# MGI-tech-bioinformatics/SuperPlus

Measured on AMD Instinct MI355X. Metric: k-mers/s (DF createDict stage: trim + canonical k-mer count + solid filter + spectrum + adjacency), higher is better.
Workload: dtype u64

## Files before the change

superplus_amd/csrc/dfk.hip:

```cpp
#include "../../include/dfk.h"
#include "dfk_kernels.h"
#include "dfk_arena.h"

#include <algorithm>
#include <chrono>
#include <cstdarg>
#include <cstdio>
#include <cstdlib>
#include <cstring>
#include <atomic>
#include <fcntl.h>
#include <functional>
#include <new>
#include <string>
#include <sys/mman.h>
#include <sys/stat.h>
#include <unistd.h>
#include <condition_variable>
#include <memory>
#include <mutex>
#include <numeric>
#include <thread>
#include <vector>

// ... 346 lines not shown
        HIP_TRY(hipStreamWaitEvent(ks, J->ev_scan, 0));
        if (step.wait_prev_count) HIP_TRY(hipStreamWaitEvent(ks, J->ev_count, 0));
    }
    HIP_TRY(hipMemsetAsync(cnt, 0, n_subs * 8, ks));
    const dim3 per_class(std::max(1u, 16u * cus / P.n_cls), P.n_cls);
    const uint32_t sh = 6 + P.sb;
    hipLaunchKernelGGL(k_keys_subcount, per_class, dim3(256), P.n_sub * 4, ks,
                       (const uint32_t*)sk.keys, (const unsigned long long*)sk.fill, sk.cap, sh, P.n_sub, cnt);
    HIP_TRY(hipGetLastError());
    hipLaunchKernelGGL(k_keys_offsets, dim3(1), dim3(1024), 0, ks, (const unsigned long long*)cnt, (uint32_t)n_subs, off, cur);
    HIP_TRY(hipGetLastError());
    hipLaunchKernelGGL(k_keys_partition, per_class, dim3(256), P.n_sub * 12, ks,
                       (const uint32_t*)sk.keys, (const unsigned long long*)sk.fill, sk.cap, sh, P.n_sub, cur, (uint32_t*)J->keys2.p);
    HIP_TRY(hipGetLastError());
    if (two) HIP_TRY(hipEventRecord(J->ev_part[sl], ks));
    ++J->n_pieces; J->count_due = true;
    if (!two) return scan_keys_count(c, T, J);
    return 0;
}

template <int K>
int scan_range(dfk_ctx* c, const Inputs& in, BucketTable* T, ScanJob* J, uint64_t r0, uint64_t r1)
{
    if (r1 <= r0) return 0;
    const PartParams& pp = J->pp;
    const ScanPlan& P = J->plan;
    const unsigned grid = scan_grid(P, r1 - r0, (unsigned)c->prop.multiProcessorCount);
    hipEvent_t e0, e1;
    HIP_TRY(hipEventCreate(&e0)); HIP_TRY(hipEventCreate(&e1));
    J->ev.emplace_back(e0, e1);
    HIP_TRY(hipEventRecord(e0, c->stream));
    if (P.keyed) {
        uint64_t p0 = r0;
        for (uint64_t m : scan_piece_sizes(P, r1 - r0, r1 == in.n_reads)) {
            int rc = scan_keys_piece<K>(c, in, T, J, p0, p0 + m); if (rc) return rc;
            p0 += m;
        }
        if (r1 == in.n_reads && J->count_due) { int rc = scan_keys_count(c, T, J); if (rc) return rc; }
    } else if (P.register_scan) {
        hipLaunchKernelGGL(HIP_KERNEL_NAME(k_scan_count<K, 16, false>), dim3(grid), dim3(PART_THREADS), scan_lds(P), c->stream,
                           in.packed, in.packed_bytes, in.base_off, (const uint32_t*)c->good_len.p, r0, r1, pp,
                           (unsigned long long*)T->acc.p, (unsigned long long*)T->class_hist.p, (unsigned long long*)J->d_n.p, P.ovf_cap,
                           (uint32_t*)J->ovf_tmp.p, (uint4*)T->summ.p, (uint32_t*)T->classes.p, ScanKeys{});
    } else {
        if (r0 != 0 || r1 != in.n_reads) return fail(DFK_E_STATE, "the general scan takes every read at once");
        hipLaunchKernelGGL(HIP_KERNEL_NAME(k_partition<K, false>), dim3(grid), dim3(PART_THREADS), scan_lds(P), c->stream,
                           in.packed, in.packed_bytes, in.base_off, (const uint32_t*)c->good_len.p, in.bc,
                           (int64_t)c->cfg.ign_bc_below, in.n_reads, pp, (unsigned long long*)T->acc.p, (unsigned long long*)T->class_hist.p,
                           (unsigned long long*)J->d_n.p, P.ovf_cap, (uint4*)J->ovf_tmp.p, (uint4*)T->summ.p,
                           (const uint32_t*)nullptr, (uint64_t)0, (const uint64_t*)nullptr, (uint32_t*)T->classes.p);
    }
    HIP_TRY(hipGetLastError());
    HIP_TRY(hipEventRecord(e1, c->stream));
    return 0;
}

template <int K>
int scan_end(dfk_ctx* c, const Inputs& in, uint64_t n_inst, BucketTable* T, ScanJob* J)
{
    int rc = 0;
    T->n_ovf = 0;
    if (J->count_due) { rc = scan_keys_count(c, T, J); if (rc) return rc; }
    c->release(J->keys); c->release(J->keys2); c->release(J->fill); c->release(J->sub);
    if (in.n_reads) {
        HIP_TRY(hipMemcpyAsync(&T->n_ovf, J->d_n.p, 8, hipMemcpyDeviceToHost, c->stream));
        HIP_TRY(hipStreamSynchronize(c->stream));
        if (T->n_ovf > J->plan.ovf_cap) {
            c->release(J->ovf_tmp);
            rc = c->alloc(J->ovf_tmp, in.n_reads * 4, "overflow read list (scratch)"); if (rc) return rc;
            HIP_TRY(hipMemsetAsync(J->d_n.p, 0, 16, c->stream));
            hipLaunchKernelGGL(k_select_overflow, dim3((unsigned)std::min<uint64_t>((in.n_reads + 255) / 256, 8192)), dim3(256), 0, c->stream,
                               (const uint4*)T->summ.p, in.n_reads, (uint32_t*)J->ovf_tmp.p, (unsigned long long*)J->d_n.p);
            HIP_TRY(hipGetLastError());
            HIP_TRY(hipMemcpyAsync(&T->n_ovf, J->d_n.p, 8, hipMemcpyDeviceToHost, c->stream));
            HIP_TRY(hipStreamSynchronize(c->stream));
        }
        if (T->n_ovf) {
            rc = c->alloc(T->ovf_list, T->n_ovf * 4, "overflow read list", Place::Low); if (rc) return rc;
            HIP_TRY(hipMemcpyAsync(T->ovf_list.p, J->ovf_tmp.p, T->n_ovf * 4, hipMemcpyDeviceToDevice, c->stream));
            HIP_TRY(hipStreamSynchronize(c->stream));
        }
    }
    c->release(J->ovf_tmp); c->release(J->d_n);
    HIP_TRY(hipStreamSynchronize(c->stream));
    float ms = 0;
    for (auto& e : J->ev) { float m = 0; if (hipEventElapsedTime(&m, e.first, e.second) == hipSuccess) ms += m; }
    c->st.ms_part_count = ms; c->st.reserved[6] = J->ev.size();
    TRACE("%llu of %llu reads have more than %d runs", (unsigned long long)T->n_ovf, (unsigned long long)in.n_reads, SUMMARY_RUNS);
    const uint64_t nb = J->plan.nb, n_bins = J->plan.n_bins;
    if (J->plan.by_class) {
        T->h_class.assign(n_bins, 0);
        HIP_TRY(hipMemcpyAsync(T->h_class.data(), T->class_hist.p, n_bins * 8, hipMemcpyDeviceToHost, c->stream));
        HIP_TRY(hipStreamSynchronize(c->stream));
        T->n_records = T->n_inst = 0;
        for (uint64_t i = 0; i < n_bins / 2; ++i) { T->n_records += T->h_class[i]; T->n_inst += T->h_class[n_bins / 2 + i]; }
    } else { rc = table_totals(c, T->acc, nb, &T->n_records, &T->n_inst); if (rc) return rc; }
    TRACE("partition count pass done (%llu buckets, %llu records%s)", (unsigned long long)nb, (unsigned long long)T->n_records, J->ev.size() > 1 ? ", in ranges under the upload" : "");
    if (T->n_inst != n_inst)
        return fail(DFK_E_HIP, "partition count pass saw %llu instances, trim saw %llu%s",
                    (unsigned long long)T->n_inst, (unsigned long long)n_inst,
                    (n_inst - T->n_inst) % (1ull << 32) == 0 ? " (a fine bucket with 2^32 or more instances: its counter keeps 32 bits)" : "");
    c->st.n_records = T->n_records; c->st.n_buckets = nb;
    return 0;
}

template <int K>
int partition_count(dfk_ctx* c, const Inputs& in, uint64_t n_inst, uint32_t log2_world, int64_t read_id0, BucketTable* T, bool by_class = false)
{
    ScanJob J;
    int rc = scan_begin<K>(c, in, log2_world, read_id0, T, by_class, &J); if (rc) return rc;
    rc = scan_range<K>(c, in, T, &J, 0, in.n_reads); if (rc) return rc;
    return scan_end<K>(c, in, n_inst, T, &J);
}

int pass_tables(dfk_ctx* c, const DevBuf& acc, uint32_t log2_sub, uint32_t world, uint32_t sub_lo, uint32_t sub_n, uint64_t budget, Partition* P)
{
    P->nb = (uint64_t)world * sub_n;
    const uint64_t nb = P->nb;
    DevBuf rec, inst, flags, idx;
    int rc = c->alloc(rec, (nb + 1) * 8, "bucket record counts"); if (rc) return rc;
    rc = c->alloc(inst, (nb + 1) * 8, "bucket instance counts"); if (rc) return rc;
    rc = c->alloc(P->base, (nb + 1) * 8, "bucket bases"); if (rc) return rc;
    rc = c->alloc(P->ipre, (nb + 1) * 8, "bucket instance prefix"); if (rc) return rc;
    const unsigned g1 = (unsigned)((nb + 1 + 255) / 256);
    hipLaunchKernelGGL(k_slice, dim3(g1), dim3(256), 0, c->stream, (const unsigned long long*)acc.p, log2_sub, sub_lo, sub_n, nb,
                       (uint64_t*)rec.p, (uint64_t*)inst.p);
    HIP_TRY(hipGetLastError());
    rc = device_scan(c, (const uint64_t*)rec.p, (uint64_t*)P->base.p, nb + 1); if (rc) return rc;
    rc = device_scan(c, (const uint64_t*)inst.p, (uint64_t*)P->ipre.p, nb + 1); if (rc) return rc;
    rc = c->alloc(flags, (nb + 1) * 8, "item flags"); if (rc) return rc;
    rc = c->alloc(idx, (nb + 1) * 8, "item index"); if (rc) return rc;
    hipLaunchKernelGGL(k_item_flags, dim3(g1), dim3(256), 0, c->stream, (const uint64_t*)P->ipre.p, nb, budget, (uint64_t*)flags.p);
    HIP_TRY(hipGetLastError());
    rc = device_scan(c, (const uint64_t*)flags.p, (uint64_t*)idx.p, nb + 1); if (rc) return rc;
    uint64_t tot[3];
    HIP_TRY(hipMemcpyAsync(&tot[0], (const uint64_t*)P->base.p + nb, 8, hipMemcpyDeviceToHost, c->stream));
    HIP_TRY(hipMemcpyAsync(&tot[1], (const uint64_t*)P->ipre.p + nb, 8, hipMemcpyDeviceToHost, c->stream));
    HIP_TRY(hipMemcpyAsync(&tot[2], (const uint64_t*)idx.p + nb, 8, hipMemcpyDeviceToHost, c->stream));
    HIP_TRY(hipStreamSynchronize(c->stream));
    P->n_records = tot[0]; P->n_inst = tot[1]; P->n_items = tot[2];
    rc = c->alloc(P->items, std::max<uint64_t>(1, P->n_items) * sizeof(ItemRange), "work items"); if (rc) return rc;
    hipLaunchKernelGGL(k_item_pairs, dim3((unsigned)((nb + 255) / 256)), dim3(256), 0, c->stream, (const uint64_t*)flags.p,
                       (const uint64_t*)idx.p, nb, (ItemRange*)P->items.p);
    HIP_TRY(hipGetLastError());
    HIP_TRY(hipStreamSynchronize(c->stream));
    c->release(rec); c->release(inst); c->release(flags); c->release(idx);
    return 0;
}

void release_pass(dfk_ctx* c, Partition* P)
{ c->release(P->records); c->release(P->base); c->release(P->ipre); c->release(P->items); }

template <int K> uint64_t item_budget(const dfk_ctx* c)
{
    constexpr uint64_t S = 1ull << CountCfg<K>::LOG2S;
    if (c->cfg.inst_per_item) return c->cfg.inst_per_item;
    if (c->distinct_per_inst <= 0.0) return 3 * S / 2;
    const double b = 0.367 * (double)S / c->distinct_per_inst;
    return (uint64_t)std::min(std::max(b, 0.5 * (double)S), 3.0 * (double)S);
}

struct ScatterJob { Partition P; DevBuf cur, d_bad; hipStream_t st = nullptr; hipEvent_t e0 = nullptr, e1 = nullptr; uint32_t lo = 0, n = 0; };

template <int K>
int scatter_launch(dfk_ctx* c, const Inputs& in, const BucketTable& T, uint32_t log2_world, int64_t read_id0, ScatterJob* J)
{
    const PartParams pp = part_params<K>(c, T.log2_nb, log2_world, read_id0, J->lo, J->n);
    HIP_TRY(hipEventRecord(J->e0, J->st));
    if (in.n_reads)
        hipLaunchKernelGGL(HIP_KERNEL_NAME(k_scatter_runs<K>), dim3((unsigned)((in.n_reads + 256ull * sweep_reads<K>() - 1) / (256ull * sweep_reads<K>()))),
                           dim3(256), 0, J->st,
// ... 1423 lines not shown
```

superplus_amd/csrc/dfk_kernels.h:

```cpp
#pragma once
#include <type_traits>
#include "dfk_device.h"
#include "dfk_fallback.h"
#include "dfk_scan_plan.h"

namespace dfk {

template <int K>
__global__ void __launch_bounds__(256)
k_trim(const uint8_t* __restrict__ pq, const uint64_t* __restrict__ pq_off, uint64_t pq_nbytes,
       const uint64_t* __restrict__ base_off, uint64_t packed_bytes, const uint32_t* __restrict__ read_len,
       uint64_t n_reads, uint32_t min_qual, uint32_t* __restrict__ good_len,
       unsigned long long* __restrict__ n_inst, unsigned int* __restrict__ bad,
       unsigned long long* __restrict__ sum_good)
{
    unsigned long long mine = 0, good = 0;
    bool any_bad = false;
    for (uint64_t r = (uint64_t)blockIdx.x * blockDim.x + threadIdx.x; r < n_reads; r += (uint64_t)gridDim.x * blockDim.x) {
        uint32_t gl = 0;
        uint64_t p = pq_off[r], end = pq_off[r + 1];
        uint32_t idx = 0, run = 0;
        const uint64_t b0 = base_off[r], b1 = base_off[r + 1];
        bool ok = p <= end && end <= pq_nbytes && b0 <= b1 && b1 <= packed_bytes && b1 - b0 >= ((uint64_t)read_len[r] + 3) / 4;
        if (!ok) end = p;
        while (p < end) {
            uint32_t nQs = pq[p];
            if (!nQs) break;
            if (p + 3 > end) { ok = false; break; }
            uint32_t hdr = pq[p + 1] | ((uint32_t)pq[p + 2] << 8);
            uint32_t nBits = hdr & 7u, minQ = (hdr >> 3) & 63u;
            uint64_t blk = ((uint64_t)nQs * nBits + 24) >> 3;
            if (p + blk > end) { ok = false; break; }
            if (nBits == 0) {
                if (minQ >= min_qual) { run += nQs; if (run >= (uint32_t)K) gl = idx + nQs; }
                else run = 0;
                idx += nQs;
            } else {
                uint64_t bit = 8 * (p + 1) + 9;
                const uint32_t fmask = (1u << nBits) - 1u;
                for (uint32_t left = nQs; left;) {
                    const uint64_t by = bit >> 3;
                    const uint32_t sh = (uint32_t)(bit & 7);
                    uint64_t w = 0;
                    if (by + 8 <= pq_nbytes) __builtin_memcpy(&w, pq + by, 8);
                    else for (uint32_t k = 0; k < 8 && by + k < pq_nbytes; ++k) w |= (uint64_t)pq[by + k] << (8 * k);
                    w >>= sh;
                    const uint32_t n = min(left, (64u - sh) / nBits);
                    for (uint32_t i = 0; i < n; ++i, w >>= nBits) {
                        const uint32_t q = minQ + ((uint32_t)w & fmask);
                        if (q < min_qual) run = 0;
                        else if (++run >= (uint32_t)K) gl = idx + 1;
                        ++idx;
                    }
                    bit += (uint64_t)n * nBits; left -= n;
                }
            }
            p += blk;
        }
        uint32_t rl = read_len[r];
        if (!ok || idx != rl) { any_bad = true; gl = 0; }
        if (gl > rl) gl = rl;
        good_len[r] = gl;
        good += gl;
        if (gl >= (uint32_t)K + 1) mine += gl - K + 1;
    }
    __shared__ unsigned long long sh[2][4];
    __shared__ unsigned int sh_bad;
    if (threadIdx.x == 0) sh_bad = 0;
    __syncthreads();
#pragma unroll
    for (int d = 32; d > 0; d >>= 1) { mine += __shfl_down(mine, d, 64); good += __shfl_down(good, d, 64); }
    if ((threadIdx.x & 63) == 0) { sh[0][threadIdx.x >> 6] = mine; sh[1][threadIdx.x >> 6] = good; }
    if (any_bad) atomicOr(&sh_bad, 1u);
    __syncthreads();
    if (threadIdx.x == 0) {
        unsigned long long a0 = sh[0][0] + sh[0][1] + sh[0][2] + sh[0][3], a1 = sh[1][0] + sh[1][1] + sh[1][2] + sh[1][3];
        if (a0) atomicAdd(n_inst, a0);
        if (a1) atomicAdd(sum_good, a1);
        if (sh_bad) atomicOr(bad, 1u);
    }
}

struct PartParams {
    uint32_t M;
    uint32_t W;
    uint32_t log2_nb;
// ... 13 lines not shown
    const uint32_t a = sweep_class_of(sub_lo, log2_local), b = sweep_class_of(sub_lo + sub_n - 1, log2_local);
    const uint32_t upto_b = b >= 31 ? 0xFFFFFFFFu : ((1u << (b + 1)) - 1u);
    return upto_b & ~((1u << a) - 1u);
}

constexpr uint32_t SUMMARY_OVERFLOW = 15;

__device__ __forceinline__ uint32_t pass_local(uint32_t bucket, const PartParams& pp)
{
    const uint32_t ls = pp.log2_nb - pp.log2_world;
    const uint32_t d = (bucket & ((1u << ls) - 1u)) - pp.sub_lo;
    return d < pp.sub_n ? (bucket >> ls) * pp.sub_n + d : 0xFFFFFFFFu;
}

__device__ __forceinline__ uint32_t bucket_of(uint32_t minhash, const PartParams& pp)
{
    const uint32_t b = (minhash * 0x9E3779B1u) >> (32 - pp.log2_nb);
    return ((b & ((1u << pp.log2_world) - 1u)) << (pp.log2_nb - pp.log2_world)) | (b >> pp.log2_world);
}
constexpr int PART_QCAP = 8;

template <int K>
__device__ __forceinline__ void emit_record(const uint32_t* __restrict__ words, uint64_t n_words, uint64_t bit0,
                                            uint32_t s0, uint32_t nk, uint32_t bucket, uint32_t gl, int32_t tag,
                                            uint64_t dst_index, uint4* __restrict__ records)
{
    const bool hp = s0 > 0;
    const bool hs = s0 + nk + (uint32_t)K <= gl;
    uint64_t bo = bit0 + 2ull * (hp ? s0 - 1 : 0);
    uint64_t wi = bo >> 5; uint32_t sh = (uint32_t)bo & 31u;
    uint32_t w[7];
#pragma unroll
    for (int i = 0; i < 7; ++i) w[i] = (wi + i < n_words) ? words[wi + i] : 0u;
    uint32_t o[6];
#pragma unroll
    for (int i = 0; i < 6; ++i) o[i] = alignbit(w[i + 1], w[i], sh);
    if (!hp) {
#pragma unroll
        for (int i = 5; i > 0; --i) o[i] = (o[i] << 2) | (o[i - 1] >> 30);
        o[0] <<= 2;
    }
    uint32_t nbits = 2u * (1u + nk + (uint32_t)K - 1u + (hs ? 1u : 0u));
#pragma unroll
    for (int i = 0; i < 6; ++i) {
        uint32_t lo = 32u * i;
        if (nbits <= lo) o[i] = 0;
        else if (nbits < lo + 32u) o[i] &= (1u << (nbits - lo)) - 1u;
    }
    uint4 a{rec_header(nk, hp, hs, bucket), (uint32_t)tag, o[0], o[1]};
    uint4 b{o[2], o[3], o[4], o[5]};
    records[2 * dst_index] = a;
    records[2 * dst_index + 1] = b;
}

__device__ __forceinline__ uint32_t class_bin(uint32_t bucket, const PartParams& pp)
{
    const uint32_t ls = pp.log2_nb - pp.log2_world;
    const uint32_t sub = bucket & ((1u << ls) - 1u);
    return (bucket >> ls) * PART_CLASSES + (ls > 6 ? sub >> (ls - 6) : sub);
}

template <int K, bool WRITE>
__device__ __forceinline__ void
partition_read(uint64_t r, uint32_t* smem, uint32_t* __restrict__ lh,
            const uint8_t* __restrict__ packed, uint64_t packed_bytes, const uint64_t* __restrict__ base_off,
            const uint32_t* __restrict__ good_len, const int32_t* __restrict__ bc, int64_t ign_bc_below,
            uint64_t n_reads, const PartParams& pp,
            unsigned long long* __restrict__ bucket_acc, unsigned long long* __restrict__ bucket_cur, uint64_t n_out,
            uint4* __restrict__ records, uint4* __restrict__ summaries, const uint32_t* __restrict__ read_list, uint64_t n_list,
            const uint64_t* __restrict__ slice_base, uint32_t* __restrict__ read_classes)
{
    auto place = [&](uint32_t b) -> uint64_t {
        if (!slice_base) { const uint64_t d = atomicAdd(&bucket_cur[b], 1ull); return d < n_out ? d : ~0ull; }
        const uint32_t owner = b / pp.sub_n;
        const uint64_t d = slice_base[owner] + atomicAdd(&bucket_cur[owner], 1ull);
        return d < slice_base[owner + 1] ? d : ~0ull;
    };
    uint32_t* arr = smem;
    uint32_t* queue = smem + pp.W * PART_THREADS;
    uint8_t* sidx = reinterpret_cast<uint8_t*>(smem + pp.W * PART_THREADS);
    uint32_t* ring = reinterpret_cast<uint32_t*>(sidx + pp.W * PART_THREADS);
    uint64_t sum_lo = 0, sum_hi = 0;
    const int tid = threadIdx.x;
    if (WRITE && read_list) { if (r >= n_list) return; r = read_list[r]; }
    const uint32_t M = pp.M, W = pp.W;
    const uint32_t gl = r < n_reads ? good_len[r] : 0;
    if (gl < (uint32_t)K + 1) {
        if (!WRITE && r < n_reads) { summaries[r] = uint4{0, 0, 0, 0}; if (read_classes) read_classes[r] = 0u; }
        return;
    }
    uint32_t Pi = 0, cur_rel = 0;
    uint32_t cmask = 0;
    const uint32_t log2_local = pp.log2_nb - pp.log2_world;

    const uint64_t byte0 = base_off[r];
    const uint32_t* words = reinterpret_cast<const uint32_t*>(packed);
    const uint64_t n_words = (packed_bytes + 3) >> 2;
    const uint64_t bit0 = byte0 * 8;
    int32_t tag = -1;
    if (bc && (int64_t)r + pp.read_id0 >= ign_bc_below) tag = bc[r];

    const uint32_t mmask = M == 16 ? 0xFFFFFFFFu : ((1u << (2 * M)) - 1u);
    const uint32_t rsh = 2 * (M - 1);
    uint32_t f = 0, rc = 0;
    uint32_t P = 0;
    uint32_t bi = 0;
    uint32_t cur_b = 0, cur_s0 = 0, cur_nk = 0;
    uint32_t qn = 0;

    uint64_t wi = bit0 >> 5;
    uint64_t filled_to = wi;
    auto fill = [&]() {
        uint32_t w[PART_RING];
#pragma unroll
        for (int k = 0; k < PART_RING; ++k) w[k] = filled_to + k < n_words ? words[filled_to + k] : 0u;
#pragma unroll
        for (int k = 0; k < PART_RING; ++k) ring[((filled_to + k) & (PART_RING - 1)) * PART_THREADS + tid] = w[k];
        filled_to += PART_RING;
    };
    uint32_t wbits, wnext = 0;
    if (!WRITE) { fill(); wbits = ring[(wi & (PART_RING - 1)) * PART_THREADS + tid]; }
    else { wbits = wi < n_words ? words[wi] : 0u; wnext = wi + 1 < n_words ? words[wi + 1] : 0u; }
    uint32_t wpos = (uint32_t)bit0 & 31u;
    uint32_t sfx_next = 0xFFFFFFFFu;

    auto close_run = [&]() {
        if (WRITE && cur_b == 0xFFFFFFFFu) return;
        if (!WRITE) {
            if (lh) { const uint32_t bin = class_bin(cur_b, pp); atomicAdd(&lh[bin], 1u); atomicAdd(&lh[(PART_CLASSES << pp.log2_world) + bin], cur_nk); }
            else atomicAdd(&bucket_acc[cur_b], (1ull << 32) | cur_nk);
            cmask |= 1u << sweep_class_of(cur_b & ((1u << log2_local) - 1u), log2_local);
            if (qn < (uint32_t)SUMMARY_RUNS) {
                const uint64_t fld = cur_nk | (cur_rel << 6);
                const uint32_t b = 8u + 12u * qn;
                if (b < 64u) { sum_lo |= fld << b; if (b > 52u) sum_hi |= fld >> (64u - b); }
                else sum_hi |= fld << (b - 64u);
            }
            ++qn;
        } else {
            if (qn == PART_QCAP) {
                for (uint32_t e = 0; e < qn; ++e) {
                    uint32_t a = queue[(2 * e) * PART_THREADS + tid], b = queue[(2 * e + 1) * PART_THREADS + tid];
                    const uint64_t dst = place(b);
                    if (dst != ~0ull) emit_record<K>(words, n_words, bit0, a & 0xFFFFu, a >> 16, b, gl, tag, dst, records);
                }
                qn = 0;
            }
            queue[(2 * qn) * PART_THREADS + tid] = cur_s0 | (cur_nk << 16);
            queue[(2 * qn + 1) * PART_THREADS + tid] = cur_b;
            ++qn;
        }
    };

    for (uint32_t j = 0; j < gl; ++j) {
        uint32_t b = (wbits >> wpos) & 3u;
        wpos += 2;
        if (wpos == 32) {
            wpos = 0; ++wi;
            if (!WRITE) { if (wi == filled_to) fill(); wbits = ring[(wi & (PART_RING - 1)) * PART_THREADS + tid]; }
            else { wbits = wnext; wnext = wi + 1 < n_words ? words[wi + 1] : 0u; }
        }
        f = ((f << 2) | b) & mmask;
        rc = (rc >> 2) | ((3u - b) << rsh);
        if (j + 1 < M) continue;
        uint32_t h = mmer_hash(f < rc ? f : rc);
        const bool newmin = bi == 0 || h < P;
        P = newmin ? h : P;
        if (!WRITE) Pi = newmin ? bi : Pi;
        const uint32_t t = j + 1 - M;
        if (t + 1 >= W) {
            uint32_t mv = P;
            bool older = false;
            if (bi != W - 1) { const uint32_t sfx = sfx_next; older = sfx < mv; mv = older ? sfx : mv; }
            const uint32_t s = t + 1 - W;
            uint32_t bucket = bucket_of(mv, pp);
            if (WRITE) bucket = pass_local(bucket, pp);
            const bool open = s == 0 || bucket != cur_b || cur_nk == (uint32_t)KTraits<K>::NK_MAX;
            if (open) {
                if (s != 0) close_run();
                cur_b = bucket; cur_s0 = s; cur_nk = 1;
                if (!WRITE) cur_rel = older ? (uint32_t)sidx[(bi + 1) * PART_THREADS + tid] - bi - 1u : W - 1u - bi + Pi;
            } else ++cur_nk;
        }
        arr[bi * PART_THREADS + tid] = h;
        if (++bi == W) {
            uint32_t run = h, ri = W - 1;
            if (!WRITE) sidx[(W - 1) * PART_THREADS + tid] = (uint8_t)(W - 1);
            for (int i0 = (int)W - 2; i0 >= 0; i0 -= 8) {
                uint32_t v[8];
#pragma unroll
                for (int k = 0; k < 8; ++k) v[k] = i0 - k >= 0 ? arr[(i0 - k) * PART_THREADS + tid] : 0u;
#pragma unroll
                for (int k = 0; k < 8; ++k) {
                    const int i = i0 - k;
                    if (i >= 0) {
                        const bool lt = v[k] < run;
                        run = lt ? v[k] : run;
                        arr[i * PART_THREADS + tid] = run;
                        if (!WRITE) { ri = lt ? (uint32_t)i : ri; sidx[i * PART_THREADS + tid] = (uint8_t)ri; }
                    }
                }
            }
            bi = 0;
        }
        if (bi + 1 < W) sfx_next = arr[(bi + 1) * PART_THREADS + tid];
    }
    close_run();
    if (!WRITE) {
        const uint64_t lo = sum_lo | (qn <= (uint32_t)SUMMARY_RUNS ? qn : SUMMARY_OVERFLOW), hi = sum_hi;
        summaries[r] = uint4{(uint32_t)lo, (uint32_t)(lo >> 32), (uint32_t)hi, (uint32_t)(hi >> 32)};
        if (read_classes) read_classes[r] = cmask;
        if (qn > (uint32_t)SUMMARY_RUNS && bucket_cur) {
            const unsigned long long at = atomicAdd(bucket_cur, 1ull);
            if (at < n_out) reinterpret_cast<uint32_t*>(records)[at] = (uint32_t)r;
        }
    }
    if (WRITE) {
        for (uint32_t e = 0; e < qn; ++e) {
            uint32_t a = queue[(2 * e) * PART_THREADS + tid], b = queue[(2 * e + 1) * PART_THREADS + tid];
            const uint64_t dst = place(b);
            if (dst != ~0ull) emit_record<K>(words, n_words, bit0, a & 0xFFFFu, a >> 16, b, gl, tag, dst, records);
        }
    }
}

template <int K, bool WRITE>
__global__ void __launch_bounds__(PART_THREADS)
k_partition(const uint8_t* __restrict__ packed, uint64_t packed_bytes, const uint64_t* __restrict__ base_off,
            const uint32_t* __restrict__ good_len, const int32_t* __restrict__ bc, int64_t ign_bc_below,
            uint64_t n_reads, PartParams pp,
            unsigned long long* __restrict__ bucket_acc,
            unsigned long long* __restrict__ class_hist,
            unsigned long long* __restrict__ bucket_cur,
            uint64_t n_out,
            uint4* __restrict__ records,
            uint4* __restrict__ summaries,
            const uint32_t* __restrict__ read_list,
            uint64_t n_list,
            const uint64_t* __restrict__ slice_base,
            uint32_t* __restrict__ read_classes)
{
    extern __shared__ uint32_t smem[];
    uint32_t* lh = nullptr;
    const uint32_t n_bins = 2u * (PART_CLASSES << pp.log2_world);
    if (!WRITE && class_hist) {
        lh = reinterpret_cast<uint32_t*>(reinterpret_cast<uint8_t*>(smem) + 5 * pp.W * PART_THREADS + 4 * PART_RING * PART_THREADS);
        for (uint32_t i = threadIdx.x; i < n_bins; i += PART_THREADS) lh[i] = 0;
        __syncthreads();
    }
    const uint64_t n_work = (WRITE && read_list) ? n_list : n_reads;
    for (uint64_t r0 = (uint64_t)blockIdx.x * PART_THREADS; r0 < n_work; r0 += (uint64_t)gridDim.x * PART_THREADS)
        partition_read<K, WRITE>(r0 + threadIdx.x, smem, lh, packed, packed_bytes, base_off, good_len, bc, ign_bc_below, n_reads, pp,
                                 bucket_acc, bucket_cur, n_out, records, summaries, read_list, n_list, slice_base, read_classes);
    if (lh) {
        __syncthreads();
        for (uint32_t i = threadIdx.x; i < n_bins; i += PART_THREADS) if (lh[i]) atomicAdd(&class_hist[i], (unsigned long long)lh[i]);
    }
}

template <int I, int N, class F>
__device__ __forceinline__ void static_for(F&& f)
{
    if constexpr (I < N) { f(std::integral_constant<int, I>{}); static_for<I + 1, N>(f); }
}

constexpr uint32_t KEY_TILE = 4096;

template <int K, int M, bool KEYS>
__global__ void __launch_bounds__(PART_THREADS)
k_scan_count(const uint8_t* __restrict__ packed, uint64_t packed_bytes, const uint64_t* __restrict__ base_off,
             const uint32_t* __restrict__ good_len, uint64_t r_first, uint64_t n_reads , PartParams pp,
             unsigned long long* __restrict__ bucket_acc, unsigned long long* __restrict__ class_hist,
             unsigned long long* __restrict__ ovf_count, uint64_t ovf_cap, uint32_t* __restrict__ ovf_list,
             uint4* __restrict__ summaries, uint32_t* __restrict__ read_classes, ScanKeys sk)
{
    constexpr int W = K - M + 1;
    constexpr uint32_t mmask = M == 16 ? 0xFFFFFFFFu : ((1u << (2 * M)) - 1u);
    constexpr uint32_t rsh = 2 * (M - 1);
    constexpr int RUNS = SUMMARY_RUNS;
    static_assert(KTraits<K>::NK_MAX < 64, "nk takes the key's six low bits");
    extern __shared__ uint32_t smem[];
    uint32_t* runb = smem;
    uint16_t* runf = reinterpret_cast<uint16_t*>(runb + RUNS * PART_THREADS);
    uint32_t* const after_runs = reinterpret_cast<uint32_t*>(runf + RUNS * PART_THREADS);
    uint32_t* lh = nullptr;
    const uint32_t n_bins = 2u * (PART_CLASSES << pp.log2_world);
    if (class_hist) {
        lh = after_runs;
        for (uint32_t i = threadIdx.x; i < n_bins; i += PART_THREADS) lh[i] = 0;
        __syncthreads();
    }
    const int tid = threadIdx.x;
    uint32_t* st_key = after_runs;
    unsigned long long* st_base = reinterpret_cast<unsigned long long*>(st_key + SCAN_STAGE);
    uint32_t* st_h = reinterpret_cast<uint32_t*>(st_base + PART_CLASSES);
    uint32_t* st_n = st_h + PART_CLASSES;
    uint8_t* st_cls = reinterpret_cast<uint8_t*>(st_n + 1);
    const uint32_t n_cls = 1u << (pp.log2_nb - sk.ib);
    if constexpr (KEYS) {
        if (tid < PART_CLASSES) st_h[tid] = 0;
        if (tid == 0) *st_n = 0;
        __syncthreads();
    }
    auto flush = [&]() {
        const uint32_t n = *st_n;
        if (tid < (int)n_cls) { const uint32_t h = st_h[tid]; if (h) st_base[tid] = atomicAdd(&sk.fill[tid], (unsigned long long)h); st_h[tid] = 0; }
        __syncthreads();
        for (uint32_t j = tid; j < n; j += PART_THREADS) {
            const uint32_t key = st_key[j], cls = st_cls[j];
            const unsigned long long at = st_base[cls] + atomicAdd(&st_h[cls], 1u);
            if (at < sk.cap) sk.keys[cls * sk.cap + at] = key;
            else atomicAdd(&bucket_acc[(cls << sk.ib) | (key >> 6)], (1ull << 32) | (key & 63u));
        }
        __syncthreads();
        if (tid < (int)n_cls) st_h[tid] = 0;
        if (tid == 0) *st_n = 0;
        __syncthreads();
    };
    const uint32_t* words = reinterpret_cast<const uint32_t*>(packed);
    const uint64_t n_words = (packed_bytes + 3) >> 2;
    const uint32_t log2_local = pp.log2_nb - pp.log2_world;
    for (uint64_t r0 = r_first + (uint64_t)blockIdx.x * PART_THREADS; r0 < n_reads; r0 += (uint64_t)gridDim.x * PART_THREADS) {
        const uint64_t r = r0 + tid;
        const uint32_t gl = r < n_reads ? good_len[r] : 0;
        const bool live = gl >= (uint32_t)K + 1;
        uint32_t qn = 0, cmask = 0;
        uint64_t sum_lo = 0, sum_hi = 0;
        if (live) {
            const uint64_t bit0 = base_off[r] * 8;
            constexpr int NW = (2 * W + 30 + 31) / 32, NA = (2 * W + 31) / 32;
            auto load = [&](uint64_t bit, uint32_t (&w)[NW]) {
                const uint64_t wi = bit >> 5;
#pragma unroll
                for (int k = 0; k < NW; ++k) {
                    const uint64_t i = wi + k;
                    const uint32_t v = words[i < n_words ? i : n_words - 1];
                    w[k] = i < n_words ? v : 0u;
                }
            };
            uint64_t nbit = bit0 + 2 * (M - 1);
            uint32_t nw[NW];
            load(nbit, nw);
            uint32_t f = 0, rc = 0;
            {
                const uint64_t wi = bit0 >> 5;
                const uint32_t w0 = words[wi < n_words ? wi : n_words - 1], w1 = words[wi + 1 < n_words ? wi + 1 : n_words - 1];
                const uint32_t pw = alignbit(wi + 1 < n_words ? w1 : 0u, wi < n_words ? w0 : 0u, (uint32_t)bit0 & 31u);
#pragma unroll
                for (int j = 0; j < M - 1; ++j) { const uint32_t b = (pw >> (2 * j)) & 3u; f = ((f << 2) | b) & mmask; rc = (rc >> 2) | ((3u - b) << rsh); }
            }
            const uint32_t n_mmers = gl - M + 1;
            uint32_t arr[W], sidxw[(W + 3) / 4];
            auto sidx_get = [&](int i) -> uint32_t { return (sidxw[i >> 2] >> (8 * (i & 3))) & 255u; };
            auto sidx_set = [&](int i, uint32_t v) { const uint32_t sh = 8u * (uint32_t)(i & 3); sidxw[i >> 2] = (sidxw[i >> 2] & ~(255u << sh)) | (v << sh); };
#pragma unroll
            for (int i = 0; i < (W + 3) / 4; ++i) sidxw[i] = 0;
            uint32_t P = 0, Pi = 0;
            uint32_t cur_b = 0, cur_nk = 0, cur_rel = 0;
            auto close_run = [&]() {
                if (qn < (uint32_t)RUNS) {
                    runb[qn * PART_THREADS + tid] = cur_b;
                    runf[qn * PART_THREADS + tid] = (uint16_t)(cur_nk | (cur_rel << 6));
                } else {
                    if (lh) { const uint32_t bin = class_bin(cur_b, pp); atomicAdd(&lh[bin], 1u); atomicAdd(&lh[(PART_CLASSES << pp.log2_world) + bin], cur_nk); }
                    else atomicAdd(&bucket_acc[cur_b], (1ull << 32) | cur_nk);
                    cmask |= 1u << sweep_class_of(cur_b & ((1u << log2_local) - 1u), log2_local);
                }
                ++qn;
            };
            for (uint32_t t0 = 0; t0 < n_mmers; t0 += W) {
                uint32_t a[NA];
                {
                    const uint32_t sh = (uint32_t)nbit & 31u;
#pragma unroll
                    for (int i = 0; i < NA; ++i) a[i] = alignbit(i + 1 < NW ? nw[i + 1] : 0u, nw[i], sh);
                }
                nbit += 2 * W;
                load(nbit, nw);
                static_for<0, W>([&](auto bi_c) {
                    constexpr int bi = decltype(bi_c)::value;
                    if (t0 + (uint32_t)bi < n_mmers) {
                        const uint32_t b = (a[(2 * bi) >> 5] >> ((2 * bi) & 31)) & 3u;
                        f = ((f << 2) | b) & mmask;
                        rc = (rc >> 2) | ((3u - b) << rsh);
                        const uint32_t h = mmer_hash(f < rc ? f : rc);
                        const bool newmin = bi == 0 || h < P;
                        P = newmin ? h : P;
                        Pi = newmin ? (uint32_t)bi : Pi;
                        const bool first = t0 == 0;
                        if (!first || bi == W - 1) {
                            uint32_t mv = P;
                            bool older = false;
                            if constexpr (bi != W - 1) { older = arr[bi + 1] < mv; mv = older ? arr[bi + 1] : mv; }
                            const uint32_t bucket = bucket_of(mv, pp);
                            const bool open = first || bucket != cur_b || cur_nk == (uint32_t)KTraits<K>::NK_MAX;
                            if (open && !first) close_run();
                            const uint32_t rel = (bi != W - 1 && older) ? sidx_get(bi + 1 < W ? bi + 1 : 0) - (uint32_t)bi - 1u : (uint32_t)(W - 1 - bi) + Pi;
                            cur_rel = open ? rel : cur_rel;
                            cur_nk = open ? 1u : cur_nk + 1u;
                            cur_b = open ? bucket : cur_b;
                        }
                        arr[bi] = h;
                        if (bi == W - 1) {
                            uint32_t run = h, ri = W - 1;
                            sidx_set(W - 1, W - 1);
                            static_for<0, W - 1>([&](auto j_c) {
                                constexpr int i = W - 2 - decltype(j_c)::value;
                                const bool lt = arr[i] < run; run = lt ? arr[i] : run; arr[i] = run; ri = lt ? (uint32_t)i : ri; sidx_set(i, ri);
                            });
                        }
                    }
                });
            }
            close_run();
        }
        const uint32_t mine = min(qn, (uint32_t)RUNS);
        for (uint32_t i = 0; KEYS ? __syncthreads_or(i < mine) != 0 : __ballot(i < mine) != 0ull; ++i) {
            const bool has = i < mine;
            uint32_t cb = 0, nk = 0;
            if (has) {
                cb = runb[i * PART_THREADS + tid];
                const uint64_t fld = runf[i * PART_THREADS + tid];
                nk = (uint32_t)fld & 63u;
                const uint32_t bfld = 8u + 12u * i;
                if (bfld < 64u) { sum_lo |= fld << bfld; if (bfld > 52u) sum_hi |= fld >> (64u - bfld); } else sum_hi |= fld << (bfld - 64u);
                if constexpr (!KEYS) {
                    if (lh) { const uint32_t bin = class_bin(cb, pp); atomicAdd(&lh[bin], 1u); atomicAdd(&lh[(PART_CLASSES << pp.log2_world) + bin], nk); }
                    else atomicAdd(&bucket_acc[cb], (1ull << 32) | nk);
                }
                cmask |= 1u << sweep_class_of(cb & ((1u << log2_local) - 1u), log2_local);
            }
            if constexpr (KEYS) {
                const uint64_t m = __ballot(has);
                if (m) {
                    const uint32_t rk = __builtin_amdgcn_mbcnt_hi((uint32_t)(m >> 32), __builtin_amdgcn_mbcnt_lo((uint32_t)m, 0u));
                    const int lead = __ffsll((unsigned long long)m) - 1;
                    uint32_t at = 0;
                    if (has && rk == 0) at = atomicAdd(st_n, (uint32_t)__popcll(m));
                    at = __shfl(at, lead) + rk;
                    if (has) {
                        const uint32_t cls = cb >> sk.ib;
                        st_key[at] = ((cb & ((1u << sk.ib) - 1u)) << 6) | nk;
                        st_cls[at] = (uint8_t)cls;
                        atomicAdd(&st_h[cls], 1u);
                    }
                }
                __syncthreads();
                if (*st_n > (uint32_t)(SCAN_STAGE - PART_THREADS)) flush();
            }
        }
        if (r < n_reads) {
            const uint64_t lo = sum_lo | (qn <= (uint32_t)SUMMARY_RUNS ? qn : SUMMARY_OVERFLOW);
            summaries[r] = uint4{(uint32_t)lo, (uint32_t)(lo >> 32), (uint32_t)sum_hi, (uint32_t)(sum_hi >> 32)};
            if (read_classes) read_classes[r] = cmask;
        }
        if (qn > (uint32_t)SUMMARY_RUNS) {
            const unsigned long long at = atomicAdd(ovf_count, 1ull);
            if (at < ovf_cap) ovf_list[at] = (uint32_t)r;
        }
    }
    if constexpr (KEYS) { __syncthreads(); if (*st_n) flush(); }
    if (lh) {
        __syncthreads();
        for (uint32_t i = threadIdx.x; i < n_bins; i += PART_THREADS) if (lh[i]) atomicAdd(&class_hist[i], (unsigned long long)lh[i]);
    }
}

constexpr int KEY_VECS = 4;
static_assert(KEY_TILE == 256u * 4u * KEY_VECS, "a tile is KEY_VECS 16-byte vectors per thread of a 256-thread block");
__device__ __forceinline__ uint32_t key_vec_n(uint64_t t0, uint64_t t1, int j)
{
    const uint64_t i = t0 + ((uint64_t)j * 256u + threadIdx.x) * 4u;
    return i < t1 ? (uint32_t)min((uint64_t)4, t1 - i) : 0u;
}
__device__ __forceinline__ void key_tile_load(const uint32_t* __restrict__ k, uint64_t t0, uint64_t t1, uint4 (&v)[KEY_VECS])
{
#pragma unroll
    for (int j = 0; j < KEY_VECS; ++j) {
        const uint64_t i = t0 + ((uint64_t)j * 256u + threadIdx.x) * 4u;
        v[j] = i < t1 ? *reinterpret_cast<const uint4*>(k + i) : make_uint4(0u, 0u, 0u, 0u);
    }
}
template <typename F>
__device__ __forceinline__ void key_tile_each(uint64_t t0, uint64_t t1, const uint4 (&v)[KEY_VECS], F&& f)
{
#pragma unroll
    for (int j = 0; j < KEY_VECS; ++j) {
        const uint32_t m = key_vec_n(t0, t1, j);
        if (m > 0) f(v[j].x);
        if (m > 1) f(v[j].y);
        if (m > 2) f(v[j].z);
        if (m > 3) f(v[j].w);
        __builtin_amdgcn_sched_barrier(0);
    }
}

__global__ void __launch_bounds__(256)
k_keys_subcount(const uint32_t* __restrict__ keys, const unsigned long long* __restrict__ fill, uint64_t cap, uint32_t sh ,
                uint32_t n_sub, unsigned long long* __restrict__ sub_cnt)
{
    extern __shared__ uint32_t lh[];
    const uint32_t c = blockIdx.y;
    for (uint32_t i = threadIdx.x; i < n_sub; i += blockDim.x) lh[i] = 0;
    __syncthreads();
    const uint64_t n = min((uint64_t)fill[c], cap);
    const uint32_t* k = keys + c * cap;
    for (uint64_t t0 = (uint64_t)blockIdx.x * KEY_TILE; t0 < n; t0 += (uint64_t)gridDim.x * KEY_TILE) {
        const uint64_t t1 = min(n, t0 + KEY_TILE);
        uint4 v[KEY_VECS];
        key_tile_load(k, t0, t1, v);
        key_tile_each(t0, t1, v, [&](uint32_t key) { atomicAdd(&lh[key >> sh], 1u); });
    }
    __syncthreads();
    for (uint32_t i = threadIdx.x; i < n_sub; i += blockDim.x) if (lh[i]) atomicAdd(&sub_cnt[(uint64_t)c * n_sub + i], (unsigned long long)lh[i]);
}

__global__ void __launch_bounds__(1024)
k_keys_offsets(const unsigned long long* __restrict__ cnt, uint32_t n, unsigned long long* __restrict__ off, unsigned long long* __restrict__ cur)
{
    __shared__ unsigned long long part[1024];
    const uint32_t tid = threadIdx.x, per = (n + 1023) / 1024;
    const uint32_t lo = min(n, tid * per), hi = min(n, lo + per);
    unsigned long long s = 0;
    for (uint32_t i = lo; i < hi; ++i) s += cnt[i];
    part[tid] = s;
    __syncthreads();
    for (uint32_t d = 1; d < 1024; d <<= 1) {
        const unsigned long long v = tid >= d ? part[tid - d] : 0ull;
        __syncthreads();
        part[tid] += v;
        __syncthreads();
    }
    unsigned long long run = part[tid] - s;
    for (uint32_t i = lo; i < hi; ++i) { off[i] = run; cur[i] = run; run += cnt[i]; }
    if (tid == 1023) off[n] = part[1023];
}

__global__ void __launch_bounds__(256)
k_keys_partition(const uint32_t* __restrict__ keys, const unsigned long long* __restrict__ fill, uint64_t cap, uint32_t sh,
                 uint32_t n_sub, unsigned long long* __restrict__ cur, uint32_t* __restrict__ out)
{
    extern __shared__ unsigned long long lds64[];
// ... 1656 lines not shown
```

Measured before the change: 64.43 billion.

## Defer bucket hashing in register scan to a post-pass fold of minimizer runs

The register-scan partition kernel now splits runs on minimizer value changes instead of computing bucket_of for every m-mer. Bucket hashing happens afterwards, once per stored run, and adjacent runs landing in the same bucket are merged by a new scan_runs_fold helper. Reads with more runs than fit in LDS, or whose fold cannot keep a valid offset, are marked overflow and recounted by a new exact pass of k_partition over the overflow list. The aim is to take hashing and branching out of the hot inner loop, at the cost of an extra kernel launch and possibly more reads taking the overflow path. Optional phase-timing instrumentation is added behind DFK_PHASE_TIMES.

```diff
diff --git a/superplus_amd/csrc/dfk.hip b/superplus_amd/csrc/dfk.hip
--- a/superplus_amd/csrc/dfk.hip
+++ b/superplus_amd/csrc/dfk.hip
@@ -452,11 +452,35 @@
         }
     }
     c->release(J->ovf_tmp); c->release(J->d_n);
+    float ms_exact = 0;
+    if (T->n_ovf && J->plan.register_scan) {
+        const ScanPlan& P = J->plan;
+        const size_t lds_b = (sizeof(uint32_t) + 1) * P.W * PART_THREADS + sizeof(uint32_t) * PART_RING * PART_THREADS + (P.by_class ? P.n_bins * 4 : 0);
+        Timer t(c->stream);
+        t.start();
+        hipLaunchKernelGGL(HIP_KERNEL_NAME(k_partition<K, false>), dim3((unsigned)std::min<uint64_t>((T->n_ovf + PART_THREADS - 1) / PART_THREADS, 1u << 20)),
+                           dim3(PART_THREADS), lds_b, c->stream,
+                           in.packed, in.packed_bytes, in.base_off, (const uint32_t*)c->good_len.p, in.bc,
+                           (int64_t)c->cfg.ign_bc_below, in.n_reads, J->pp, (unsigned long long*)T->acc.p, (unsigned long long*)T->class_hist.p,
+                           (unsigned long long*)nullptr, (uint64_t)0, (uint4*)nullptr, (uint4*)nullptr,
+                           (const uint32_t*)T->ovf_list.p, T->n_ovf, (const uint64_t*)nullptr, (uint32_t*)T->classes.p);
+        HIP_TRY(hipGetLastError());
+        ms_exact = t.stop();
+    }
     HIP_TRY(hipStreamSynchronize(c->stream));
-    float ms = 0;
+#ifdef DFK_PHASE_TIMES
+    {
+        unsigned long long ph[4] = {};
+        (void)hipMemcpyFromSymbol(ph, HIP_SYMBOL(g_scan_phase), sizeof ph);
+        const double tot = (double)(ph[0] + ph[1] + ph[2]);
+        fprintf(stderr, "[dfk] scan wave ticks (since the process began): base loop %.3e (%.1f %%), fold of the runs %.3e (%.1f %%), per-run loop and summaries %.3e (%.1f %%)\n",
+                (double)ph[0], 100.0 * ph[0] / tot, (double)ph[1], 100.0 * ph[1] / tot, (double)ph[2], 100.0 * ph[2] / tot);
+    }
+#endif
+    float ms = ms_exact;
     for (auto& e : J->ev) { float m = 0; if (hipEventElapsedTime(&m, e.first, e.second) == hipSuccess) ms += m; }
     c->st.ms_part_count = ms; c->st.reserved[6] = J->ev.size();
-    TRACE("%llu of %llu reads have more than %d runs", (unsigned long long)T->n_ovf, (unsigned long long)in.n_reads, SUMMARY_RUNS);
+    TRACE("%llu of %llu reads have more runs than the %d of a summary", (unsigned long long)T->n_ovf, (unsigned long long)in.n_reads, SUMMARY_RUNS);
     const uint64_t nb = J->plan.nb, n_bins = J->plan.n_bins;
     if (J->plan.by_class) {
         T->h_class.assign(n_bins, 0);
diff --git a/superplus_amd/csrc/dfk_kernels.h b/superplus_amd/csrc/dfk_kernels.h
--- a/superplus_amd/csrc/dfk_kernels.h
+++ b/superplus_amd/csrc/dfk_kernels.h
@@ -2,6 +2,7 @@
 #include <type_traits>
 #include "dfk_device.h"
 #include "dfk_fallback.h"
+#include "dfk_scan_runs.h"
 #include "dfk_scan_plan.h"
 
 namespace dfk {
@@ -181,11 +182,11 @@
     uint32_t* ring = reinterpret_cast<uint32_t*>(sidx + pp.W * PART_THREADS);
     uint64_t sum_lo = 0, sum_hi = 0;
     const int tid = threadIdx.x;
-    if (WRITE && read_list) { if (r >= n_list) return; r = read_list[r]; }
+    if (read_list) { if (r >= n_list) return; r = read_list[r]; }
     const uint32_t M = pp.M, W = pp.W;
     const uint32_t gl = r < n_reads ? good_len[r] : 0;
     if (gl < (uint32_t)K + 1) {
-        if (!WRITE && r < n_reads) { summaries[r] = uint4{0, 0, 0, 0}; if (read_classes) read_classes[r] = 0u; }
+        if (!WRITE && r < n_reads) { if (summaries) summaries[r] = uint4{0, 0, 0, 0}; if (read_classes) read_classes[r] = 0u; }
         return;
     }
     uint32_t Pi = 0, cur_rel = 0;
@@ -307,7 +308,7 @@
     close_run();
     if (!WRITE) {
         const uint64_t lo = sum_lo | (qn <= (uint32_t)SUMMARY_RUNS ? qn : SUMMARY_OVERFLOW), hi = sum_hi;
-        summaries[r] = uint4{(uint32_t)lo, (uint32_t)(lo >> 32), (uint32_t)hi, (uint32_t)(hi >> 32)};
+        if (summaries) summaries[r] = uint4{(uint32_t)lo, (uint32_t)(lo >> 32), (uint32_t)hi, (uint32_t)(hi >> 32)};
         if (read_classes) read_classes[r] = cmask;
         if (qn > (uint32_t)SUMMARY_RUNS && bucket_cur) {
             const unsigned long long at = atomicAdd(bucket_cur, 1ull);
@@ -347,7 +348,7 @@
         for (uint32_t i = threadIdx.x; i < n_bins; i += PART_THREADS) lh[i] = 0;
         __syncthreads();
     }
-    const uint64_t n_work = (WRITE && read_list) ? n_list : n_reads;
+    const uint64_t n_work = read_list ? n_list : n_reads;
     for (uint64_t r0 = (uint64_t)blockIdx.x * PART_THREADS; r0 < n_work; r0 += (uint64_t)gridDim.x * PART_THREADS)
         partition_read<K, WRITE>(r0 + threadIdx.x, smem, lh, packed, packed_bytes, base_off, good_len, bc, ign_bc_below, n_reads, pp,
                                  bucket_acc, bucket_cur, n_out, records, summaries, read_list, n_list, slice_base, read_classes);
@@ -364,6 +365,13 @@
 }
 
 constexpr uint32_t KEY_TILE = 4096;
+
+#ifdef DFK_PHASE_TIMES
+__device__ unsigned long long g_scan_phase[4];
+#define SCAN_PH(i) do { const unsigned long long ph_n = __builtin_amdgcn_s_memtime(); if ((tid & 63) == 0) atomicAdd(&g_scan_phase[i], ph_n - ph_t); ph_t = ph_n; } while (0)
+#else
+#define SCAN_PH(i) do { } while (0)
+#endif
 
 template <int K, int M, bool KEYS>
 __global__ void __launch_bounds__(PART_THREADS)
@@ -381,6 +389,8 @@
     extern __shared__ uint32_t smem[];
     uint32_t* runb = smem;
     uint16_t* runf = reinterpret_cast<uint16_t*>(runb + RUNS * PART_THREADS);
+    uint8_t* const run_bytes = reinterpret_cast<uint8_t*>(smem);
+    constexpr uint32_t RUNF_AT = sizeof(uint32_t) * RUNS * PART_THREADS;
     uint32_t* const after_runs = reinterpret_cast<uint32_t*>(runf + RUNS * PART_THREADS);
     uint32_t* lh = nullptr;
     const uint32_t n_bins = 2u * (PART_CLASSES << pp.log2_world);
@@ -425,7 +435,12 @@
         const bool live = gl >= (uint32_t)K + 1;
         uint32_t qn = 0, cmask = 0;
         uint64_t sum_lo = 0, sum_hi = 0;
+#ifdef DFK_PHASE_TIMES
+        unsigned long long ph_t = __builtin_amdgcn_s_memtime();
+#endif
         if (live) {
+            uint32_t slot = 2u * (uint32_t)tid;
+            const uint32_t slot_end = slot + 2u * PART_THREADS * RUNS;
             const uint64_t bit0 = base_off[r] * 8;
             constexpr int NW = (2 * W + 30 + 31) / 32, NA = (2 * W + 31) / 32;
             auto load = [&](uint64_t bit, uint32_t (&w)[NW]) {
@@ -455,17 +470,13 @@
 #pragma unroll
             for (int i = 0; i < (W + 3) / 4; ++i) sidxw[i] = 0;
             uint32_t P = 0, Pi = 0;
-            uint32_t cur_b = 0, cur_nk = 0, cur_rel = 0;
+            uint32_t cur_mv = 0, cur_nk = 0, cur_rel = 0;
             auto close_run = [&]() {
-                if (qn < (uint32_t)RUNS) {
-                    runb[qn * PART_THREADS + tid] = cur_b;
-                    runf[qn * PART_THREADS + tid] = (uint16_t)(cur_nk | (cur_rel << 6));
-                } else {
-                    if (lh) { const uint32_t bin = class_bin(cur_b, pp); atomicAdd(&lh[bin], 1u); atomicAdd(&lh[(PART_CLASSES << pp.log2_world) + bin], cur_nk); }
-                    else atomicAdd(&bucket_acc[cur_b], (1ull << 32) | cur_nk);
-                    cmask |= 1u << sweep_class_of(cur_b & ((1u << log2_local) - 1u), log2_local);
+                if (slot < slot_end) {
+                    *reinterpret_cast<uint32_t*>(run_bytes + 2u * slot) = cur_mv;
+                    *reinterpret_cast<uint16_t*>(run_bytes + RUNF_AT + slot) = (uint16_t)(cur_nk | (cur_rel << 6));
                 }
-                ++qn;
+                slot += 2u * PART_THREADS;
             };
             for (uint32_t t0 = 0; t0 < n_mmers; t0 += W) {
                 uint32_t a[NA];
@@ -491,13 +502,14 @@
                             uint32_t mv = P;
                             bool older = false;
                             if constexpr (bi != W - 1) { older = arr[bi + 1] < mv; mv = older ? arr[bi + 1] : mv; }
-                            const uint32_t bucket = bucket_of(mv, pp);
-                            const bool open = first || bucket != cur_b || cur_nk == (uint32_t)KTraits<K>::NK_MAX;
-                            if (open && !first) close_run();
-                            const uint32_t rel = (bi != W - 1 && older) ? sidx_get(bi + 1 < W ? bi + 1 : 0) - (uint32_t)bi - 1u : (uint32_t)(W - 1 - bi) + Pi;
-                            cur_rel = open ? rel : cur_rel;
-                            cur_nk = open ? 1u : cur_nk + 1u;
-                            cur_b = open ? bucket : cur_b;
+                            const bool open = first || mv != cur_mv || cur_nk == (uint32_t)KTraits<K>::NK_MAX;
+                            if (open) {
+                                if (!first) close_run();
+                                cur_rel = (bi != W - 1 && older) ? sidx_get(bi + 1 < W ? bi + 1 : 0) - (uint32_t)bi - 1u : (uint32_t)(W - 1 - bi) + Pi;
+                                cur_nk = 0;
+                                cur_mv = mv;
+                            }
+                            ++cur_nk;
                         }
                         arr[bi] = h;
                         if (bi == W - 1) {
@@ -512,8 +524,28 @@
                 });
             }
             close_run();
-        }
-        const uint32_t mine = min(qn, (uint32_t)RUNS);
+            qn = (slot - 2u * (uint32_t)tid) / (2u * PART_THREADS);
+        }
+        SCAN_PH(0);
+        bool exact = qn > (uint32_t)RUNS;
+        if (qn != 0 && !exact) {
+            bool fold = false;
+            uint32_t prev = 0;
+            for (uint32_t j = 0; j < qn; ++j) {
+                const uint32_t b = bucket_of(runb[j * PART_THREADS + tid], pp);
+                runb[j * PART_THREADS + tid] = b;
+                fold = fold || (j != 0 && b == prev);
+                prev = b;
+            }
+            if (fold) {
+                const int m = scan_runs_fold(runb + tid, runf + tid, (uint32_t)PART_THREADS, qn, (uint32_t)KTraits<K>::NK_MAX,
+                                             [](uint32_t b) { return b; });
+                exact = m < 0;
+                qn = (uint32_t)m;
+            }
+        }
+        SCAN_PH(1);
+        const uint32_t mine = exact ? 0u : qn;
         for (uint32_t i = 0; KEYS ? __syncthreads_or(i < mine) != 0 : __ballot(i < mine) != 0ull; ++i) {
             const bool has = i < mine;
             uint32_t cb = 0, nk = 0;
@@ -549,14 +581,15 @@
             }
         }
         if (r < n_reads) {
-            const uint64_t lo = sum_lo | (qn <= (uint32_t)SUMMARY_RUNS ? qn : SUMMARY_OVERFLOW);
+            const uint64_t lo = sum_lo | (exact ? SUMMARY_OVERFLOW : qn);
             summaries[r] = uint4{(uint32_t)lo, (uint32_t)(lo >> 32), (uint32_t)sum_hi, (uint32_t)(sum_hi >> 32)};
             if (read_classes) read_classes[r] = cmask;
         }
-        if (qn > (uint32_t)SUMMARY_RUNS) {
+        if (exact) {
             const unsigned long long at = atomicAdd(ovf_count, 1ull);
             if (at < ovf_cap) ovf_list[at] = (uint32_t)r;
         }
+        SCAN_PH(2);
     }
     if constexpr (KEYS) { __syncthreads(); if (*st_n) flush(); }
     if (lh) {
diff --git a/superplus_amd/csrc/dfk_scan_runs.h b/superplus_amd/csrc/dfk_scan_runs.h
--- /dev/null
+++ b/superplus_amd/csrc/dfk_scan_runs.h
@@ -0,0 +1,39 @@
+#pragma once
+#include <cstdint>
+
+#if defined(__HIPCC__) || defined(__CUDACC__)
+#define DFK_SCAN_RUNS_HD __host__ __device__ __forceinline__
+#else
+#define DFK_SCAN_RUNS_HD inline
+#endif
+
+namespace dfk {
+
+template <class BucketOf>
+DFK_SCAN_RUNS_HD int scan_runs_fold(uint32_t* key, uint16_t* fld, uint32_t stride, uint32_t n, uint32_t nk_max, BucketOf&& bucket_of)
+{
+    uint32_t out = 0;
+    uint32_t b = 0, onk = 0, orel = 0;
+    bool bad = false;
+    for (uint32_t j = 0; j < n; ++j) {
+        const uint32_t bj = bucket_of(key[j * stride]);
+        const uint32_t f = fld[j * stride], nkj = f & 63u, relj = f >> 6;
+        if (onk != 0 && bj != b) {
+            key[out * stride] = b; fld[out * stride] = (uint16_t)(onk | (orel << 6)); ++out; onk = 0;
+        }
+        b = bj;
+        if (onk == 0) orel = relj;
+        const uint32_t room = nk_max - onk, take = nkj < room ? nkj : room;
+        onk += take;
+        if (onk == nk_max) {
+            key[out * stride] = b; fld[out * stride] = (uint16_t)(onk | (orel << 6)); ++out;
+            onk = nkj - take;
+            bad = bad || (onk != 0 && relj < take);
+            orel = relj - take;
+        }
+    }
+    if (onk != 0) { key[out * stride] = b; fld[out * stride] = (uint16_t)(onk | (orel << 6)); ++out; }
+    return bad ? -1 : (int)out;
+}
+
+}
```

After: 64.96 billion, median of 6. About the same (+0.8%).
